# afanasyev-ilya/VectorGraphLibrary

Measured on AMD Instinct MI355X. Metric: TEPS (edges/s) BFS + SSSP on RMAT-24; value = direction-optimising BFS, sssp_value_teps = direction-optimising Bellman-Ford, higher is better.
Workload: dtype int32; 1 GPU; BFS direction-optimising on RMAT scale-24 (edge factor 32), 1xMI355X; vertices=16777216, edges=536870912, seed=1, parallelism=edge-cut x1, exchange_transport=none, vertex_numbering=degree-sorted (total)

## Files before the change

include/vgl_hip.h:

```cpp
#ifndef VGL_HIP_H
#define VGL_HIP_H
#include <stddef.h>
#include <stdint.h>
#ifdef __cplusplus
extern "C" {
#endif

#define VGL_HIP_ABI_VERSION 1

typedef struct vgl_hip_ctx vgl_hip_ctx;
typedef struct vgl_hip_graph vgl_hip_graph;
typedef struct vgl_hip_frontier vgl_hip_frontier;

int vgl_hip_abi_version(void);
const char *vgl_hip_last_error(void);
int vgl_hip_ctx_create(int device, void *stream, vgl_hip_ctx **out);
int vgl_hip_ctx_destroy(vgl_hip_ctx *ctx);
int vgl_hip_ctx_sync(vgl_hip_ctx *ctx);
int vgl_hip_ctx_trim(vgl_hip_ctx *ctx);
void *vgl_hip_ctx_stream(vgl_hip_ctx *ctx);

int vgl_hip_malloc(vgl_hip_ctx *ctx, size_t bytes, void **dptr);
int vgl_hip_free(vgl_hip_ctx *ctx, void *dptr);
int vgl_hip_memcpy_h2d(vgl_hip_ctx *ctx, void *dst, const void *src, size_t bytes);
// ... 267 lines not shown
    int64_t undirected_edges;
    int64_t components;
    int64_t bridges;
    int64_t articulation_points;
    int64_t biconnected_components;
    int64_t two_edge_components;
    int64_t largest_component_edges;
    int64_t algorithmic_bytes;
} vgl_hip_bicc_stats;
int vgl_hip_bicc_prepare(vgl_hip_ctx *ctx, vgl_hip_graph *g, int64_t *undirected_edges);
int vgl_hip_bicc_run(vgl_hip_ctx *ctx, vgl_hip_graph *g, int32_t *d_edge_u, int32_t *d_edge_v, uint8_t *d_bridge, int32_t *d_edge_component,
                     uint8_t *d_articulation, int32_t *d_two_edge_component, vgl_hip_bicc_stats *stats);

int vgl_hip_bfs_init(vgl_hip_ctx *ctx, int32_t V, int32_t source, int32_t *d_levels);
int vgl_hip_bfs_step_top_down(vgl_hip_ctx *ctx, vgl_hip_graph *g, int32_t *d_levels, int32_t level,
                              const uint64_t *d_visited_bits, int64_t *local_frontier, int64_t *local_edges);
int vgl_hip_bfs_step_top_down_bits(vgl_hip_ctx *ctx, vgl_hip_graph *graph, int32_t *d_levels, int32_t level,
                                   const uint64_t *d_visited_bits, const uint64_t *d_front_bits, uint64_t *d_next_bits,
                                   int64_t *local_frontier, int64_t *local_edges);
int vgl_hip_bitmap_or_parts(vgl_hip_ctx *ctx, int64_t words, int parts, const uint64_t *d_in, uint64_t *d_out);
int vgl_hip_bfs_step_bottom_up(vgl_hip_ctx *ctx, vgl_hip_graph *g, int32_t *d_levels, int32_t level,
                               const uint64_t *d_visited_bits, const uint64_t *d_front_bits, uint64_t *d_next_bits,
                               int64_t *found, int64_t *probed);
int vgl_hip_levels_to_bitmap(vgl_hip_ctx *ctx, int32_t V, const int32_t *d_levels, int32_t level, uint64_t *d_bits);
int vgl_hip_bfs_apply_bitmaps(vgl_hip_ctx *ctx, int32_t V, int parts, const uint64_t *d_bits_all, int32_t *d_levels, int32_t level,
                              uint64_t *d_visited_bits, uint64_t *d_front_bits, const int32_t *d_degrees, int64_t *newly,
                              int64_t *newly_degree);
int vgl_hip_bfs_apply_bitmaps_owned(vgl_hip_ctx *ctx, int32_t V, int parts, const uint64_t *d_bits_all, int32_t *d_levels, int32_t level,
                                    uint64_t *d_visited_bits, uint64_t *d_front_bits, const int32_t *d_degrees, int32_t own_begin,
                                    int32_t own_end, int64_t *newly_owned, int64_t *newly_owned_degree);
int vgl_hip_bitmap_to_ids(vgl_hip_ctx *ctx, int64_t words, const uint64_t *d_bits, int32_t cap, int32_t *d_out);
int vgl_hip_bfs_apply_ids(vgl_hip_ctx *ctx, int32_t V, int parts, int32_t cap, const int32_t *d_lists, int32_t *d_levels, int32_t level,
                          uint64_t *d_visited_bits, uint64_t *d_front_bits, const int32_t *d_degrees, int64_t *newly,
                          int64_t *newly_degree);
int vgl_hip_sssp_init(vgl_hip_ctx *ctx, int32_t V, int32_t source, float *d_dist);
int vgl_hip_sssp_relax_owned(vgl_hip_ctx *ctx, vgl_hip_graph *g, const float *d_weights, float *d_dist, int *changed);
int vgl_hip_cc_init(vgl_hip_ctx *ctx, int32_t V, int32_t *d_comp);
int vgl_hip_cc_hook_owned(vgl_hip_ctx *ctx, vgl_hip_graph *g, int32_t *d_comp, int *changed);
int vgl_hip_cc_jump(vgl_hip_ctx *ctx, int32_t V, int32_t *d_comp);
int vgl_hip_pr_setup(vgl_hip_ctx *ctx, int32_t V, const int32_t *d_indeg_noloops, float *d_ranks, float *d_rdeg);
int vgl_hip_sum_over_edges_f32(vgl_hip_ctx *ctx, vgl_hip_graph *g, const float *d_values, float sum_bound, float *d_sums);
int vgl_hip_pr_iteration_owned(vgl_hip_ctx *ctx, vgl_hip_graph *g, const int32_t *d_indeg_noloops, const float *d_rdeg,
                               float *d_ranks, float *d_contrib_scratch);
int vgl_hip_diff_to_pairs_u32(vgl_hip_ctx *ctx, int32_t n, const void *d_before, const void *d_after, int32_t cap, int32_t *d_out);
int vgl_hip_apply_pairs_u32(vgl_hip_ctx *ctx, int parts, int64_t stride, int skip_part, const int32_t *d_lists, int take_min, int32_t n,
                            void *d_values, int *changed);
// ... 55 lines not shown
```

vectorgraphlibrary_amd/api.py:

```python
import ctypes as C

import torch

from . import lib as _l

RMAT_ABCD = (57, 19, 19, 5)
BFS_TOP_DOWN, BFS_DIRECTION_OPT = 0, 1
SSSP_ALL_ACTIVE, SSSP_ACTIVE_TILES, SSSP_DELTA_STEPPING, SSSP_PULL, SSSP_DIRECTION_OPT = 0, 1, 2, 3, 4
DENSE, SPARSE, ALL_ACTIVE = 0, 1, 2
PR_EXACT_ORDER, PR_BLOCKED, PR_AUTO = 0, 1, 2
LP_ALL_ACTIVE, LP_FRONTIER, LP_AUTO = 0, 1, 2


def _ptr(t):
    return C.c_void_p(t.data_ptr()) if t is not None else None


class Context:

    def __init__(self, device=0):
        if not torch.cuda.is_available():
            raise _l.VglHipError("no HIP device visible: vectorgraphlibrary_amd has no CPU fallback")
        self.L = _l.load()
        self.device = torch.device("cuda", device)
# ... 4 lines not shown
        self.h = h

    def sync(self):
        _l.check(self.L.vgl_hip_ctx_sync(self.h))

    def close(self):
        if self.h:
            self.L.vgl_hip_ctx_destroy(self.h)
            self.h = None

    def empty(self, n, dtype):
        return torch.empty(int(n), dtype=dtype, device=self.device)

    def timing(self, enable=True, only=None, stride=1):
        _l.check(self.L.vgl_hip_timing_enable(self.h, int(enable)))
        _l.check(self.L.vgl_hip_timing_only(self.h, only.encode() if only else None))
        _l.check(self.L.vgl_hip_timing_stride(self.h, int(stride)))
        _l.check(self.L.vgl_hip_timing_reset(self.h))

    def timing_get(self, name):
        n, ms = C.c_int64(), C.c_double()
        _l.check(self.L.vgl_hip_timing_get(self.h, name.encode(), C.byref(n), C.byref(ms)))
        return n.value, ms.value

    def gen_rmat(self, scale, edge_factor, seed, relabel=True, first_edge=0, count=None):
        E = (1 << scale) * edge_factor if count is None else count
        src, dst = self.empty(E, torch.int32), self.empty(E, torch.int32)
        a, b, c, d = RMAT_ABCD
        _l.check(self.L.vgl_hip_gen_rmat(self.h, scale, first_edge, E, seed, a, b, c, d, int(relabel), _ptr(src), _ptr(dst)))
        return src, dst

    def gen_uniform(self, scale, edge_factor, seed, first_edge=0, count=None):
        E = (1 << scale) * edge_factor if count is None else count
        src, dst = self.empty(E, torch.int32), self.empty(E, torch.int32)
        _l.check(self.L.vgl_hip_gen_uniform(self.h, scale, first_edge, E, seed, _ptr(src), _ptr(dst)))
        return src, dst

    def gen_weights(self, E, seed, first_edge=0):
        w = self.empty(E, torch.float32)
        _l.check(self.L.vgl_hip_gen_weights(self.h, first_edge, E, seed, _ptr(w)))
        return w

    def coo_to_csr(self, V, src, dst, row_begin=0, row_end=None, want_perm=False):
        row_end = V if row_end is None else row_end
        E = src.numel()
        rowptr = self.empty(row_end - row_begin + 1, torch.int64)
# ... 627 lines not shown
```

vectorgraphlibrary_amd/csrc/bfs.hip:

```cpp
#include "vgl_hip_internal.h"
#include <chrono>
#include "vgl_gnf.h"
#include "vgl_blocked.h"

#ifndef VGL_BU_HEAVY_LANES
#define VGL_BU_HEAVY_LANES 16
#endif

__global__ __launch_bounds__(VGL_BLOCK) void vgl_k_bfs_init(int32_t V, int32_t source, int32_t *levels)
{
    for (int32_t v = blockIdx.x * VGL_BLOCK + threadIdx.x; v < V; v += gridDim.x * VGL_BLOCK)
        levels[v] = (v == source) ? 1 : -1;
}

__global__ __launch_bounds__(VGL_BLOCK) void vgl_k_bfs_init_all(int32_t V, int32_t source, int32_t *levels, int64_t words, uint64_t *visited,
                                                                uint64_t *front, uint64_t *next, uint32_t *tickets, unsigned long long *list_count)
{
    if (blockIdx.x == 0 && threadIdx.x == 0) *list_count = 0ULL;
    for (int32_t v = blockIdx.x * VGL_BLOCK + threadIdx.x; v < V; v += gridDim.x * VGL_BLOCK)
        levels[v] = (v == source) ? 1 : -1;
    for (int64_t w = (int64_t)blockIdx.x * VGL_BLOCK + threadIdx.x; w < words; w += (int64_t)gridDim.x * VGL_BLOCK) {
        const uint64_t bit = (w == (source >> 6)) ? (1ULL << (source & 63)) : 0ULL;
        visited[w] = bit; front[w] = bit; next[w] = 0;
    }
// ... 603 lines not shown
        host[C_NSLOTS] = seq;
        __threadfence_system();
    }
}

constexpr int VGL_BU_BLOCKS = 2048;

typedef int vgl_int4_u __attribute__((ext_vector_type(4), aligned(4)));

typedef unsigned vgl_uint3_u __attribute__((ext_vector_type(3), aligned(4)));
template <bool PACKED>
__device__ __forceinline__ void vgl_load_head(const int4 *in_head, int64_t rec, int32_t u[4])
{
    if constexpr (PACKED) {
        const vgl_uint3_u w = *reinterpret_cast<const vgl_uint3_u *>(reinterpret_cast<const uint32_t *>(in_head) + 3 * rec);
        const uint32_t f[4] = {w.x & 0xFFFFFFu, (w.x >> 24) | ((w.y & 0xFFFFu) << 8), (w.y >> 16) | ((w.z & 0xFFu) << 16), w.z >> 8};
#pragma unroll
        for (int q = 0; q < 4; q++) u[q] = f[q] == 0xFFFFFFu ? -1 : (int32_t)f[q];
    } else {
        const int4 h = in_head[rec];
        u[0] = h.x; u[1] = h.y; u[2] = h.z; u[3] = h.w;
    }
}
template <bool INLINE_HEAVY, bool PACKED>
__device__ __forceinline__ void vgl_bu_probe_body(int32_t nrows, int32_t row_base, int32_t chunk, const int64_t *in_rowptr,
                                                  const int32_t *in_adj, const uint64_t *visited, const uint64_t *in_nz,
                                                  const uint64_t *front, uint64_t *next, int32_t *levels, int32_t next_level,
                                                  int32_t *heavy, int64_t *partials, uint32_t *ticket, const int4 *in_head,
                                                  const uint64_t *in_long, const int32_t *nz_rank, int32_t nz_rows, int64_t *counters,
                                                  volatile int64_t *host, int64_t seq)
{
    static_assert(INLINE_HEAVY, "the deferred rows are scanned in the same launch");
    __shared__ int64_t s64[VGL_WAVES];
    __shared__ int s_nheavy;
    if (threadIdx.x == 0) s_nheavy = 0;
    __syncthreads();
    auto in_front = [&](int32_t u) -> uint32_t { return (uint32_t)((front[u >> 6] >> (u & 63)) & 1ULL); };
    int64_t found_cnt = 0, probes = 0;
    const int64_t groups = ((int64_t)nrows + 63) >> 6;
    const int64_t word0 = (int64_t)row_base >> 6;
    constexpr int64_t NW = (int64_t)VGL_BU_BLOCKS * VGL_WAVES;
    int32_t *my_heavy = heavy + (int64_t)blockIdx.x * chunk;
    const int lane = vgl_lane();
    for (int64_t g0 = (int64_t)blockIdx.x * VGL_WAVES + vgl_wave(); g0 < groups; g0 += NW * 64) {
        const int64_t mine = g0 + (int64_t)lane * NW;
        uint64_t cw = 0, nzw = 0;
        int32_t nzr = 0;
        if (mine < groups) {
            nzw = in_nz[word0 + mine];
            cw = ~visited[word0 + mine] & nzw;
            if (cw == 0ULL) next[word0 + mine] = 0ULL;
            else nzr = nz_rank[mine];
        }
        unsigned long long todo = __ballot(cw != 0ULL);
        while (todo) {
            const int j = __ffsll((long long)todo) - 1;
            todo &= todo - 1;
            const uint64_t cand_word = __shfl(cw, j);
            const int32_t rec = __shfl(nzr, j) + (int32_t)__popcll(__shfl(nzw, j) & ((1ULL << lane) - 1ULL));
            const int64_t grp = g0 + (int64_t)j * NW;
            const int32_t r = (int32_t)(grp << 6) + lane;
            const int32_t v = row_base + r;
            bool found = false, defer = false;
            if (r < nrows && ((cand_word >> lane) & 1ULL)) {
                int32_t u0[4];
                vgl_load_head<PACKED>(in_head, rec, u0);
                uint32_t hit = 0;
                int n = 0;
#pragma unroll
                for (int q = 0; q < 4; q++) if (u0[q] >= 0) n = q + 1;
                if (u0[0] >= 0) hit = in_front(u0[0]);
                if (hit == 0) {
#pragma unroll
                    for (int q = 1; q < 4; q++)
                        if (u0[q] >= 0) hit |= in_front(u0[q]) << q;
                }
                bool longer = false;
                if (hit == 0 && n == 4) {
                    int32_t u1[4];
                    vgl_load_head<PACKED>(in_head, (int64_t)nz_rows + rec, u1);
#pragma unroll
                    for (int q = 0; q < 4; q++)
                        if (u1[q] >= 0) { n = 5 + q; hit |= in_front(u1[q]) << (4 + q); }
                    longer = (in_long[v >> 6] >> (v & 63)) & 1ULL;
                }
                found = hit != 0;
                probes += found ? __ffs(hit) : n;
                defer = !found && longer;
                if (found) levels[v] = next_level;
            }
            const unsigned long long fm = __ballot(found);
            if (lane == 0) next[word0 + grp] = fm;
            found_cnt += found;
            const unsigned long long dm = __ballot(defer);
            if (dm) {
                int base = 0;
                if (lane == 0) base = atomicAdd(&s_nheavy, (int)__popcll(dm));
                base = __shfl(base, 0);
                if (defer) my_heavy[base + __popcll(dm & ((1ULL << lane) - 1ULL))] = r;
            }
        }
    }
    __syncthreads();
    const int nh = s_nheavy;
    constexpr int G = VGL_BU_HEAVY_LANES, NG = 64 / G;
    const int quarter = lane / G, ql = lane % G;
    for (int h0 = vgl_wave() * NG; h0 < nh; h0 += VGL_WAVES * NG) {
        const int h = h0 + quarter;
        bool done = h >= nh, hit_any = false;
        int32_t r = 0;
        int64_t p = 0, e = 0;
        if (!done) { r = my_heavy[h]; p = in_rowptr[r]; e = in_rowptr[r + 1]; }
        while (!__all(done)) {
            const int64_t q = p + ql;
            bool hit = false;
            if (!done && q < e) { const int32_t u = in_adj[q]; hit = (front[u >> 6] >> (u & 63)) & 1ULL; }
            const unsigned long long hm = __ballot(hit);
            const unsigned qm = (unsigned)(hm >> (quarter * G)) & (G >= 32 ? 0xFFFFFFFFu : ((1u << (G & 31)) - 1u));
            if (!done) {
                if (qm) { hit_any = true; done = true; if (ql == 0) probes += __ffs(qm); }
                else { if (ql == 0) probes += min((int64_t)G, e - p); p += G; if (p >= e) done = true; }
            }
        }
        if (hit_any && ql == 0) {
            const int32_t v = row_base + r;
            levels[v] = next_level;
            atomicOr((unsigned long long *)&next[v >> 6], 1ULL << (v & 63));
            found_cnt++;
        }
    }
    found_cnt = vgl_block_reduce_add(found_cnt, s64);
    probes = vgl_block_reduce_add(probes, s64);
    uint32_t dep = 0;
    if (threadIdx.x == 0) dep = vgl_put_agent(partials + blockIdx.x * 4 + 0, found_cnt) ^ vgl_put_agent(partials + blockIdx.x * 4 + 1, probes);
    if (!vgl_last_block(ticket, dep)) return;
    int64_t f = 0, pr = 0;
    for (int b = threadIdx.x; b < (int)gridDim.x; b += VGL_BLOCK) { f += vgl_load_agent(partials + b * 4 + 0); pr += vgl_load_agent(partials + b * 4 + 1); }
    f = vgl_block_reduce_add(f, s64);
    pr = vgl_block_reduce_add(pr, s64);
    if (threadIdx.x == 0) {
        if (host) vgl_publish2(counters, host, seq, C_BU_FOUND, f, C_BU_EDGES, pr);
        else { counters[C_BU_FOUND] = f; counters[C_BU_EDGES] = pr; }
    }
}
#define VGL_BU_PROBE_PARAMS                                                                                                                             \
    int32_t nrows, int32_t row_base, int32_t chunk, const int64_t *in_rowptr, const int32_t *in_adj, const uint64_t *visited, const uint64_t *in_nz,  \
        const uint64_t *front, uint64_t *next, int32_t *levels, int32_t next_level, int32_t *heavy, int64_t *partials, uint32_t *ticket,               \
        const int4 *in_head, const uint64_t *in_long, const int32_t *nz_rank, int32_t nz_rows, int64_t *counters, volatile int64_t *host, int64_t seq
#define VGL_BU_PROBE_ARGS                                                                                                                               \
    nrows, row_base, chunk, in_rowptr, in_adj, visited, in_nz, front, next, levels, next_level, heavy, partials, ticket, in_head, in_long, nz_rank,    \
        nz_rows, counters, host, seq
template <bool INLINE_HEAVY>
__global__ __launch_bounds__(VGL_BLOCK) __attribute__((amdgpu_num_sgpr(80))) void vgl_k_bu_probe(VGL_BU_PROBE_PARAMS)
{
    vgl_bu_probe_body<INLINE_HEAVY, true>(VGL_BU_PROBE_ARGS);
}
template <bool INLINE_HEAVY>
__global__ __launch_bounds__(VGL_BLOCK) void vgl_k_bu_probe_wide(VGL_BU_PROBE_PARAMS)
{
    vgl_bu_probe_body<INLINE_HEAVY, false>(VGL_BU_PROBE_ARGS);
}

__global__ __launch_bounds__(VGL_BLOCK) void vgl_k_bm_advance(int64_t words, uint64_t *visited, uint64_t *front, uint64_t *next)
{
    for (int64_t w = (int64_t)blockIdx.x * VGL_BLOCK + threadIdx.x; w < words; w += (int64_t)gridDim.x * VGL_BLOCK) {
        const uint64_t n = next[w];
        if (n) { visited[w] |= n; next[w] = 0; }
        front[w] = n;
    }
}

constexpr int VGL_B2I_BLOCKS = 2048;
__global__ __launch_bounds__(VGL_BLOCK) void vgl_k_bitmap_to_ids(int64_t words, const uint64_t *bits, int64_t word_base, int32_t cap, int32_t *out)
{
    __shared__ int s32[VGL_WAVES];
    __shared__ int s_base;
    const int64_t per = (((words + gridDim.x - 1) / gridDim.x + VGL_BLOCK - 1) / VGL_BLOCK) * VGL_BLOCK;
    const int64_t lo = (int64_t)blockIdx.x * per, hi = min(words, lo + per);
    int n = 0;
    for (int64_t wi = lo + threadIdx.x; wi < hi; wi += VGL_BLOCK) n += (int)__popcll(bits[wi]);
    int total = 0;
    vgl_block_excl_add(n, s32, &total);
    if (total == 0) return;
    if (threadIdx.x == 0) s_base = atomicAdd(out, total);
// ... 156 lines not shown
            if (advance)
                hipLaunchKernelGGL(vgl_k_bm_gnf_count<true>, dim3(nb), dim3(VGL_BLOCK), 0, c->stream, nwords, word0, g->row_begin, g->bm_front,
                                   g->out.rowptr, g->vt_cnt, g->vt_deg, g->vt_cnt_off, g->vt_deg_off, g->offs, c->d_counters,
                                   g->tickets + 0 * VGL_TICKET_WORDS, (volatile int64_t *)c->h_counters, seq, g->bm_visited, g->bm_next,
                                   hint ? 1 : 0, hint ? *hint : no_hint);
            else
                hipLaunchKernelGGL(vgl_k_bm_gnf_count<false>, dim3(nb), dim3(VGL_BLOCK), 0, c->stream, nwords, word0, g->row_begin,
                                   const_cast<uint64_t *>(front), g->out.rowptr, g->vt_cnt, g->vt_deg, g->vt_cnt_off, g->vt_deg_off, g->offs, c->d_counters,
                                   g->tickets + 0 * VGL_TICKET_WORDS, (volatile int64_t *)c->h_counters, seq, (uint64_t *)nullptr, (uint64_t *)nullptr,
                                   0, no_hint);
        }
        VGL_HIP_TRY(hipGetLastError());
        VGL_TRY(vgl_wait_counters(c, seq));
    }
    if (write) {
        vgl_timed_launch tl(c, "gnf");
        hipLaunchKernelGGL(vgl_k_bm_gnf_write, dim3(nb), dim3(VGL_BLOCK), 0, c->stream, nwords, word0, g->row_begin, front,
                           g->out.rowptr, g->vt_cnt_off, g->vt_deg_off, g->ids, g->offs, g->tile_first, M_known >= 0 ? M_known : c->h_counters[C_NEIGH]);
        VGL_HIP_TRY(hipGetLastError());
    }
    return 0;
}

static int vgl_bfs_bu_launch(vgl_hip_ctx *c, vgl_hip_graph *g, int32_t *levels, int32_t next_level, const uint64_t *visited,
                             const uint64_t *front, uint64_t *next, int64_t *seq_out)
{
    const int32_t chunk = (int32_t)(vgl_ceil_div(vgl_ceil_div(g->nrows, VGL_BU_BLOCKS), VGL_BLOCK) * VGL_BLOCK);
    const int64_t seq = vgl_next_seq(c);
    {
        vgl_timed_launch tl(c, "bfs_bottom_up");
        auto *kernel = g->in_head_packed ? vgl_k_bu_probe<true> : vgl_k_bu_probe_wide<true>;
        hipLaunchKernelGGL(kernel, dim3(VGL_BU_BLOCKS), dim3(VGL_BLOCK), 0, c->stream, g->nrows, g->row_begin, chunk,
                           g->in.rowptr, g->in.adj, visited, g->bm_in_nz, front, next, levels, next_level, g->heavy, g->bu_partials,
                           g->tickets + 1 * VGL_TICKET_WORDS, reinterpret_cast<const int4 *>(g->in_head.p), g->bm_in_long,
                           (const int32_t *)g->in_nz_rank, g->in_nz_rows, c->d_counters, (volatile int64_t *)c->h_counters, seq);
    }
    VGL_HIP_TRY(hipGetLastError());
    if (seq_out) *seq_out = seq;
    return 0;
}

static int vgl_bfs_blocked_level(vgl_hip_ctx *c, vgl_hip_graph *g, int32_t *levels, int32_t next_level)
{
    for (const vgl_blocked_piece &p : g->blk_bfs->pieces) {
        if (p.n_g_units > 0) {
            vgl_timed_launch tl(c, "bfs_blk_gather");
            hipLaunchKernelGGL(vgl_k_bfs_blk_gather, dim3((unsigned)p.n_g_units), dim3(VGL_BTHREADS), 0, c->stream, (const vgl_blk_unit *)p.g_units,
                               (const uint16_t *)p.g_lo, (const uint32_t *)p.mid_to_a, reinterpret_cast<uint64_t *>(p.vals.p), p.g_count,
                               (const uint64_t *)g->bm_front, (int64_t)g->row_begin >> 6);
        }
        if (p.n_a_units > 0) {
            vgl_timed_launch tl(c, "bfs_blk_accumulate");
// ... 19 lines not shown
}

int vgl_bitmap_to_ids(vgl_hip_ctx *c, int64_t words, const uint64_t *d_bits, int64_t word_base, int32_t cap, int32_t *d_out)
{
    VGL_HIP_TRY(hipMemsetAsync(d_out, 0, sizeof(int32_t), c->stream));
    if (words > 0) {
        vgl_timed_launch tl(c, "bfs_shard_resolve");
        hipLaunchKernelGGL(vgl_k_bitmap_to_ids, dim3((unsigned)std::min<int64_t>(VGL_B2I_BLOCKS, vgl_ceil_div(words, VGL_BLOCK))), dim3(VGL_BLOCK), 0, c->stream,
                           words, d_bits, word_base, cap, d_out);
    }
    VGL_HIP_TRY(hipGetLastError());
    return 0;
}

static int64_t vgl_bfs_td_emit_edges(int64_t V) { return std::max<int64_t>(65536, V / 256); }

struct vgl_bfs_params {
    int64_t td_emit_edges;
    double td_filter_share;
    double td_late_share;
    double blocked_share;
    int64_t small_m;
    int64_t bm_expand_f;
    bool use_hints, scan_bound, trace;
};
static vgl_bfs_params vgl_bfs_params_of(const vgl_bfs_tunables &tn, int64_t V, int mode)
{
    const bool do_mode = mode == VGL_HIP_BFS_DIRECTION_OPT;
    vgl_bfs_params p;
    p.td_emit_edges = tn.td_emit_edges >= 0 ? tn.td_emit_edges : vgl_bfs_td_emit_edges(V);
    p.td_filter_share = tn.td_filter_share >= 0.0 ? tn.td_filter_share : 0.125;
    p.td_late_share = tn.td_late_share >= 0.0 ? tn.td_late_share : 1.0 / 64;
    p.blocked_share = tn.blocked_share >= 0.0 ? tn.blocked_share : 0.1;
    p.small_m = tn.small_m >= 0 ? std::min<int64_t>(tn.small_m, 1 << 20) : 8192;
    if (do_mode) p.small_m = std::min<int64_t>(p.small_m, vgl_do_bottom_up_edges(V, V, 1) - 1);
    if (p.small_m < 64) p.small_m = 0;
    p.bm_expand_f = tn.bm_expand >= 0 ? tn.bm_expand : 262144;
    if (vgl_ceil_div(vgl_ceil_div(V, 64), VGL_BLOCK) > 8192) p.bm_expand_f = 0;
    p.use_hints = do_mode && !tn.no_hint;
    p.scan_bound = do_mode && !tn.no_scan_bound;
    p.trace = tn.trace;
    return p;
}

enum class vgl_bfs_front {
    levels,
    pending,
    bitmap,
    counted_bitmap,
    counted_scan,
    ids,
};

struct vgl_bfs_traversal {
    vgl_hip_ctx *c;
    vgl_hip_graph *g;
    int mode;
    int32_t *levels;
    vgl_bfs_params p;
    int32_t V;
    int64_t E, words, factor;
// ... 157 lines not shown
            VGL_TRY(small_levels((int32_t)F, -1, false));
            trace("list kernel done");
            book_small(F);
            return 0;
        }
        const bool is_late = late();
        const bool emit = M <= p.td_emit_edges || is_late;
        const bool td_counts = emit && p.use_hints && vgl_ceil_div(M, VGL_TILE) <= VGL_TD_COUNT_TILES;
        const bool filter = is_late || (double)visited_total >= p.td_filter_share * (double)V;
        trace(emit ? "counted + ids -> top-down (emitting)" : "counted + ids -> top-down (levels only)");
        VGL_TRY(vgl_bfs_td_launch(c, g, (int32_t)F, M, levels, cur + 1, emit, have_tile_first, td_counts, filter));
        trace("top-down done");
        hint_ready = td_counts && F > 0 && M > 0;
        front = emit ? vgl_bfs_front::pending : vgl_bfs_front::levels;
        book_top_down(F, M);
        cur++;
        return 0;
    }
    int bottom_up_level()
    {
        if (front == vgl_bfs_front::levels || front == vgl_bfs_front::pending) VGL_FAIL("bfs_run: internal error (bitmaps missing)");
        int64_t seq = 0;
        trace("-> bottom-up");
        VGL_TRY(vgl_bfs_bu_launch(c, g, levels, cur + 1, g->bm_visited, g->bm_front, g->bm_next, &seq));
        hipLaunchKernelGGL(vgl_k_bm_advance, dim3(vgl_grid(words, VGL_BLOCK, 8192)), dim3(VGL_BLOCK), 0, c->stream, words, g->bm_visited, g->bm_front, g->bm_next);
        VGL_HIP_TRY(hipGetLastError());
        VGL_TRY(vgl_wait_counters(c, seq));
        st.bu_steps++; st.edges_examined += c->h_counters[C_BU_EDGES];
        st.bu_edges += c->h_counters[C_BU_EDGES]; st.bu_found += c->h_counters[C_BU_FOUND];
        F = c->h_counters[C_BU_FOUND]; M = 0;
        front = vgl_bfs_front::bitmap;
        cur++;
        return 0;
    }

    int run(int32_t source)
    {
        hipLaunchKernelGGL(vgl_k_bfs_init_all, dim3(vgl_grid(V, VGL_BLOCK, 8192)), dim3(VGL_BLOCK), 0, c->stream, V, source, levels, words, g->bm_visited, g->bm_front,
                           g->bm_next, g->tickets, list_count);
        t0 = std::chrono::steady_clock::now();
        if (p.small_m > 0) {
            VGL_TRY(small_levels(1, source, false));
            if (c->h_counters[C_TMP0] > 0) {
                begin_level(1);
                prevF = 1;
                book_small(1);
            }
// ... 121 lines not shown
        vgl_timed_launch tl(c, "gnf");
        hipLaunchKernelGGL(vgl_k_levels_to_bitmap<false>, dim3(vgl_grid(g->V, VGL_BLOCK, 8192)), dim3(VGL_BLOCK), 0, c->stream, g->V, (const int32_t *)d_levels, level + 1, d_next_bits);
    }
    VGL_HIP_TRY(hipGetLastError());
    return 0;
}

int vgl_hip_bfs_step_bottom_up(vgl_hip_ctx *c, vgl_hip_graph *g, int32_t *d_levels, int32_t level, const uint64_t *d_visited_bits,
                               const uint64_t *d_front_bits, uint64_t *d_next_bits, int64_t *found, int64_t *probed)
{
    if (!c || !g || !d_levels || !d_visited_bits || !d_front_bits || !d_next_bits) VGL_FAIL("bfs_step_bottom_up: null argument");
    if (!g->in.rowptr) VGL_FAIL("bfs_step_bottom_up: the incoming CSR of the owned rows is required");
    VGL_TRY(vgl_zero_words(c, d_next_bits, vgl_ceil_div(g->V, 64)));
    int64_t seq = 0;
    VGL_TRY(vgl_bfs_bu_launch(c, g, d_levels, level + 1, d_visited_bits, d_front_bits, d_next_bits, &seq));
    if (found || probed) {
        VGL_TRY(vgl_wait_counters(c, seq));
        if (found) *found = c->h_counters[C_BU_FOUND];
        if (probed) *probed = c->h_counters[C_BU_EDGES];
    }
    return 0;
}

int vgl_hip_bitmap_or_parts(vgl_hip_ctx *c, int64_t words, int parts, const uint64_t *d_in, uint64_t *d_out)
{
    if (!c || !d_in || !d_out) VGL_FAIL("bitmap_or_parts: null argument");
    if (words < 0 || parts < 1) VGL_FAIL("bitmap_or_parts: bad size");
    if (words > 0) hipLaunchKernelGGL(vgl_k_bitmap_or_parts, dim3(vgl_grid(words, VGL_BLOCK, 8192)), dim3(VGL_BLOCK), 0, c->stream, words, parts, d_in, d_out);
    VGL_HIP_TRY(hipGetLastError());
    return 0;
}

int vgl_hip_levels_to_bitmap(vgl_hip_ctx *c, int32_t V, const int32_t *d_levels, int32_t level, uint64_t *d_bits)
{
    if (!c || !d_levels || !d_bits) VGL_FAIL("levels_to_bitmap: null argument");
    hipLaunchKernelGGL(vgl_k_levels_to_bitmap<false>, dim3(vgl_grid(V, VGL_BLOCK, 8192)), dim3(VGL_BLOCK), 0, c->stream, V, d_levels, level, d_bits);
    VGL_HIP_TRY(hipGetLastError());
    return 0;
}

int vgl_hip_bitmap_to_ids(vgl_hip_ctx *c, int64_t words, const uint64_t *d_bits, int32_t cap, int32_t *d_out)
{
    if (!c || !d_bits || !d_out) VGL_FAIL("bitmap_to_ids: null argument");
    if (words < 0 || cap < 1) VGL_FAIL("bitmap_to_ids: bad size");
    return vgl_bitmap_to_ids(c, words, d_bits, 0, cap, d_out);
}
// ... 63 lines not shown
```

vectorgraphlibrary_amd/csrc/context.hip:

```cpp
#include "vgl_hip_internal.h"
#include <unordered_set>
#include <cstdio>
#include <cstring>
#include <mutex>
#include <algorithm>

static thread_local std::string g_last_error;

int vgl_set_error(const char *file, int line, const char *msg)
{
    char buf[512];
    const char *base = strrchr(file, '/');
    snprintf(buf, sizeof(buf), "vgl_hip: %s (%s:%d)", msg, base ? base + 1 : file, line);
    g_last_error = buf;
    return 1;
}

static hipMemPool_t g_lib_pool[64];
static bool g_lib_pool_tried[64];
static std::mutex g_lib_pool_mutex;
hipMemPool_t vgl_lib_pool(int device)
{
    if (device < 0 || device >= 64) return nullptr;
    std::lock_guard<std::mutex> lock(g_lib_pool_mutex);
// ... 29 lines not shown
extern char **environ;
static uint64_t vgl_env_signature()
{
    uint64_t h = 1469598103934665603ull ^ (uint64_t)(uintptr_t)environ;
    if (environ) for (char **e = environ; *e; e++) h = (h ^ (uint64_t)(uintptr_t)*e) * 1099511628211ull;
    return h ? h : 1;
}
void vgl_ctx_refresh_env(vgl_hip_ctx *c)
{
    const uint64_t sig = vgl_env_signature();
    if (sig == c->env_signature) return;
    c->env_signature = sig;
    c->env.clear();
    if (environ)
        for (char **e = environ; *e; e++)
            if (strncmp(*e, "VGL_", 4) == 0)
                if (const char *eq = strchr(*e, '=')) c->env[std::string(*e, (size_t)(eq - *e))] = std::string(eq + 1);
    vgl_bfs_tunables t;
    auto str = [&](const char *n) -> const char * { auto it = c->env.find(n); return it == c->env.end() ? nullptr : it->second.c_str(); };
    auto on = [&](const char *n) { const char *v = str(n); return v && v[0] == '1'; };
    if (const char *v = str("VGL_TD_EMIT_EDGES")) t.td_emit_edges = atoll(v);
    if (const char *v = str("VGL_BFS_SMALL_M")) t.small_m = atoll(v);
    if (const char *v = str("VGL_BFS_BM_EXPAND")) t.bm_expand = atoll(v);
    if (const char *v = str("VGL_SHARD_TD_EMIT_EDGES")) t.shard_td_emit_edges = atoll(v);
    if (const char *v = str("VGL_TD_FILTER_SHARE")) t.td_filter_share = atof(v);
    if (const char *v = str("VGL_TD_LATE_SHARE")) t.td_late_share = atof(v);
    if (const char *v = str("VGL_BFS_BLOCKED_SHARE")) t.blocked_share = atof(v);
    if (const char *v = str("VGL_SHARD_SPARSE_CAP")) t.shard_sparse_cap = std::max(0, atoi(v));
    t.no_hint = on("VGL_BFS_NO_HINT"); t.no_scan_bound = on("VGL_BFS_NO_SCAN_BOUND"); t.trace = on("VGL_BFS_TRACE");
    c->bfs = t;
}
const char *vgl_env(vgl_hip_ctx *c, const char *name)
{
    vgl_ctx_refresh_env(c);
    auto it = c->env.find(name);
    return it == c->env.end() ? nullptr : it->second.c_str();
}
int64_t vgl_env_int(vgl_hip_ctx *c, const char *name, int64_t dflt, int64_t lo, int64_t hi)
{
    const char *s = vgl_env(c, name);
    const int64_t v = (s && *s) ? strtoll(s, nullptr, 10) : dflt;
    return std::min(hi, std::max(lo, v));
}

extern "C" {

// ... 241 lines not shown
```

vectorgraphlibrary_amd/csrc/graph_frontier.hip:

```cpp
#include "vgl_hip_internal.h"
#include <atomic>
#include "vgl_gnf.h"
#include "vgl_blocked.h"

__global__ __launch_bounds__(VGL_BLOCK) void vgl_k_tile_rows(int32_t nrows, const int64_t *rowptr, int32_t *tile_row, int64_t ntiles)
{
    for (int32_t r = blockIdx.x * VGL_BLOCK + threadIdx.x; r < nrows; r += gridDim.x * VGL_BLOCK) {
        const int64_t t0 = (rowptr[r] + VGL_TILE - 1) / VGL_TILE;
        const int64_t t1 = (rowptr[r + 1] + VGL_TILE - 1) / VGL_TILE;
        for (int64_t t = t0; t < t1; t++) tile_row[t] = r;
        if (rowptr[r] < rowptr[r + 1] && rowptr[r + 1] == rowptr[nrows]) tile_row[ntiles] = r;
    }
}

__global__ __launch_bounds__(VGL_BLOCK) void vgl_k_nonempty_rows(int32_t nrows, int32_t row_base, const int64_t *rowptr, uint64_t *bits)
{
    const int32_t nround = (nrows + 63) & ~63;
    for (int32_t r = blockIdx.x * VGL_BLOCK + threadIdx.x; r < nround; r += gridDim.x * VGL_BLOCK) {
        const bool on = r < nrows && rowptr[r + 1] > rowptr[r];
        const unsigned long long m = __ballot(on);
        if ((threadIdx.x & 63) == 0) bits[(row_base + r) >> 6] = m;
    }
}

// ... 259 lines not shown
                         const int64_t *d_in_rowptr, const int32_t *d_in_adj, int64_t in_edges, vgl_hip_graph **out)
{
    if (!c || !out) VGL_FAIL("graph_create: null argument");
    if (V <= 0) VGL_FAIL("graph_create: vertices_count must be positive");
    if (row_begin < 0 || row_end > V || row_begin >= row_end) VGL_FAIL("graph_create: bad owned row range");
    if (row_begin % 64 != 0) VGL_FAIL("graph_create: row_begin must be a multiple of 64 (use vgl_hip_partition_rows)");
    if (!d_out_rowptr || (!d_out_adj && out_edges > 0)) VGL_FAIL("graph_create: outgoing CSR is required");
    if (out_edges < 0 || in_edges < 0) VGL_FAIL("graph_create: negative edge count");
    VGL_HIP_TRY(hipSetDevice(c->device));
    vgl_building<vgl_hip_graph> g(new vgl_hip_graph(), {c});
    static std::atomic<uint64_t> next_uid{1};
    g->uid = next_uid.fetch_add(1);
    g->V = V; g->row_begin = row_begin; g->row_end = row_end; g->nrows = row_end - row_begin;
    g->out.rowptr = d_out_rowptr; g->out.adj = d_out_adj; g->out.edges = out_edges;
    VGL_TRY(vgl_build_tile_rows(c, g->out, g->nrows));
    if (d_in_rowptr) {
        g->in.rowptr = d_in_rowptr; g->in.adj = d_in_adj; g->in.edges = in_edges;
        VGL_TRY(vgl_build_tile_rows(c, g->in, g->nrows));
    }
    const size_t words = (size_t)vgl_ceil_div(V, 64) + 1;
    VGL_TRY(g->bm_visited.alloc(words));
    VGL_TRY(g->bm_front.alloc(words));
    VGL_TRY(g->bm_next.alloc(words));
    VGL_TRY(g->bm_in_nz.alloc(words));
    VGL_TRY(g->ids.alloc((size_t)g->nrows));
    VGL_TRY(g->offs.alloc((size_t)g->nrows + 1));
    g->nvtiles = vgl_ceil_div(g->nrows, VGL_TILE);
    VGL_TRY(g->vt_cnt.alloc((size_t)g->nvtiles));
    VGL_TRY(g->vt_cnt_off.alloc((size_t)g->nvtiles));
    VGL_TRY(g->vt_deg.alloc((size_t)g->nvtiles));
    VGL_TRY(g->vt_deg_off.alloc((size_t)g->nvtiles));
    VGL_TRY(g->vt_min_deg.alloc((size_t)g->nvtiles));
    hipLaunchKernelGGL(vgl_k_tile_min_degree, dim3((unsigned)g->nvtiles), dim3(VGL_BLOCK), 0, c->stream, g->nrows, g->out.rowptr, g->vt_min_deg);
    VGL_TRY(g->tile_first.alloc((size_t)g->out.ntiles + 2));
    VGL_TRY(g->heavy.alloc((size_t)g->nrows + 4096 * VGL_BLOCK));
    VGL_TRY(g->bu_partials.alloc((size_t)4096 * 4));
    VGL_TRY(g->tickets.alloc((size_t)4 * VGL_TICKET_WORDS));
    VGL_HIP_TRY(hipMemsetAsync(g->tickets, 0, 4 * VGL_TICKET_WORDS * sizeof(uint32_t), c->stream));
    VGL_TRY(g->epoch.alloc((size_t)V));
    VGL_TRY(g->fscratch.alloc((size_t)V));
    VGL_TRY(g->fscratch2.alloc((size_t)V));
    VGL_TRY(g->fscratch3.alloc((size_t)V));
    VGL_TRY(g->iscratch.alloc((size_t)V));
    VGL_HIP_TRY(hipMemsetAsync(g->bm_visited, 0, words * 8, c->stream));
    VGL_HIP_TRY(hipMemsetAsync(g->bm_front, 0, words * 8, c->stream));
    VGL_HIP_TRY(hipMemsetAsync(g->bm_next, 0, words * 8, c->stream));
// ... 351 lines not shown
```

vectorgraphlibrary_amd/csrc/vgl_hip_internal.h:

```cpp
#pragma once
#include <hip/hip_runtime.h>
#include <stdint.h>
#include <string>
#include <map>
#include <memory>
#include <vector>
#include "../../include/vgl_hip.h"

constexpr int VGL_BLOCK = 256;
constexpr int VGL_EPT = 8;
constexpr int VGL_TILE = VGL_BLOCK * VGL_EPT;
constexpr int VGL_WAVES = VGL_BLOCK / 64;

int vgl_set_error(const char *file, int line, const char *msg);
#define VGL_FAIL(msg) return vgl_set_error(__FILE__, __LINE__, (msg))
#define VGL_HIP_TRY(expr)                                                          \
    do {                                                                           \
        hipError_t _e = (expr);                                                    \
        if (_e != hipSuccess) return vgl_set_error(__FILE__, __LINE__, hipGetErrorString(_e)); \
    } while (0)
#define VGL_TRY(expr)            \
    do {                         \
        int _s = (expr);         \
        if (_s != 0) return _s;  \
    } while (0)

enum {
    C_FRONT = 0, C_NEIGH = 1, C_BU_FOUND = 2, C_BU_EDGES = 3, C_HEAVY = 4, C_CHANGED = 5,
    C_EDGES = 6, C_TMP0 = 7, C_TMP1 = 8, C_JUMP = 9,
    C_NEXT_F = 10, C_NEXT_M = 11,
    C_SKIPPED = 12, C_HINT = 13,
    C_NSLOTS = 32
};
constexpr int VGL_NSHARD = 1024;

struct vgl_timing_slot {
    int64_t launches = 0;
    std::vector<std::pair<hipEvent_t, hipEvent_t>> pending;
    double total_ms = 0.0;
};

struct vgl_bfs_tunables {
    int64_t td_emit_edges = -1, small_m = -1, bm_expand = -1, shard_td_emit_edges = -1;
    double td_filter_share = -1.0, td_late_share = -1.0, blocked_share = -1.0;
    int shard_sparse_cap = -1;
    bool no_hint = false, no_scan_bound = false, trace = false;
};

struct vgl_hip_ctx {
    std::map<std::string, std::string> env;
    uint64_t env_signature = 0;
    vgl_bfs_tunables bfs;
    int device = 0;
    hipStream_t stream = nullptr;
    bool own_stream = false;
    int64_t *d_counters = nullptr;
    int64_t *d_shards = nullptr;
    int64_t *h_counters = nullptr;
    int64_t publish_seq = 0;
    double *d_partials = nullptr;
    size_t partials_cap = 0;
    bool timing = false;
    std::string timing_only;
    int timing_stride = 1;
    int64_t timing_seen = 0;
    std::map<std::string, vgl_timing_slot> slots;
// ... 75 lines not shown
    vgl_dev<int32_t> tile_row;
    int64_t ntiles = 0;
    vgl_dev<int32_t> hub_rows;
    int32_t nhubs = 0;
    int hub_blocks = 0;
    vgl_dev<int32_t> giant_rows;
    int ngiants = 0, giant_blocks = 0;
    vgl_dev<int32_t> hub_chunks;
    int n_hub_chunks = 0, n_hub_list = 0;
    vgl_dev<double> hub_chunk_sums;
    vgl_dev<int32_t> pull_blk_row;
    int pull_nblk = 0;
    int64_t max_row = -1;
};

template <class T> void vgl_cache_free(T *p);
template <class T> struct vgl_cache_delete { void operator()(T *p) const { vgl_cache_free(p); } };
template <class T> using vgl_cache = std::unique_ptr<T, vgl_cache_delete<T>>;
struct vgl_hip_graph {
    uint64_t uid = 0;
    int32_t V = 0, row_begin = 0, row_end = 0, nrows = 0;
    vgl_dir_csr out, in;
    vgl_dev<uint64_t> bm_visited, bm_front, bm_next;
    vgl_dev<uint64_t> bm_in_nz;
    vgl_dev<int32_t> in_head;
    bool in_head_packed = false;
    vgl_dev<int32_t> in_nz_rank;
    int32_t in_nz_rows = 0;
    vgl_dev<int32_t> pr_indeg;
    bool pr_indeg_ready = false;
    vgl_dev<uint64_t> bm_in_long;
    vgl_dev<int32_t> ids;
    vgl_dev<int64_t> offs;
    vgl_dev<int32_t> vt_cnt, vt_cnt_off;
    vgl_dev<int64_t> vt_deg, vt_deg_off;
    int64_t nvtiles = 0;
    vgl_dev<int32_t> vt_min_deg;
    vgl_dev<uint8_t> gnf_bits;
    vgl_dev<int32_t> tile_first;
    vgl_dev<int32_t> heavy;
    vgl_dev<int64_t> bu_partials;
    vgl_dev<uint32_t> tickets;
    vgl_dev<int32_t> epoch;
    vgl_dev<float> fscratch;
    vgl_dev<float> fscratch2;
    vgl_dev<float> fscratch3;
// ... 259 lines not shown
```

vectorgraphlibrary_amd/lib.py:

```python
import ctypes as C
import os

_HERE = os.path.dirname(os.path.abspath(__file__))
LIB_PATH = os.path.join(_HERE, "libvgl_hip.so")


class VglHipError(RuntimeError):
    pass


class BfsStats(C.Structure):
    _fields_ = [("levels", C.c_int32), ("td_steps", C.c_int32), ("bu_steps", C.c_int32),
                ("edges_examined", C.c_int64), ("frontier_total", C.c_int64), ("discovered", C.c_int64),
                ("algorithmic_bytes", C.c_int64), ("td_edges", C.c_int64), ("td_frontier", C.c_int64),
                ("bu_edges", C.c_int64), ("bu_found", C.c_int64)]


class SsspStats(C.Structure):
    _fields_ = [("iterations", C.c_int32), ("edges_relaxed", C.c_int64), ("algorithmic_bytes", C.c_int64),
                ("push_steps", C.c_int32), ("pull_steps", C.c_int32)]


class PrStats(C.Structure):
    _fields_ = [("iterations", C.c_int32), ("ranks_sum", C.c_double), ("algorithmic_bytes", C.c_int64)]
# ... 129 lines not shown
    "vgl_hip_cc_run": [_p, _p, _p, C.POINTER(CcStats)],
    "vgl_hip_cc_run_symmetric": [_p, _p, _p, C.POINTER(CcStats)],
    "vgl_hip_lp_prepare": [_p, _p, _int],
    "vgl_hip_lp_run": [_p, _p, _int, _int, _int, _int, _p, _p, C.POINTER(_i64), C.POINTER(LpStats)],
    "vgl_hip_tri_prepare": [_p, _p],
    "vgl_hip_tri_run": [_p, _p, C.POINTER(_i64), _p, _p, C.POINTER(TriStats)],
    "vgl_hip_bc_prepare": [_p, _p, _int],
    "vgl_hip_bc_run": [_p, _p, C.POINTER(_i32), _i32, _int, _int, _p, _p, _p, _p, C.POINTER(BcStats)],
    "vgl_hip_msbfs_prepare": [_p, _p, _int, _int],
    "vgl_hip_msbfs_run": [_p, _p, C.POINTER(_i32), _i32, _int, _int, _p, _p, _p, _p, _p, C.POINTER(MsbfsStats)],
    "vgl_hip_kcore_prepare": [_p, _p],
    "vgl_hip_kcore_run": [_p, _p, _i32, _p, _p, C.POINTER(KcoreStats)],
    "vgl_hip_ktruss_prepare": [_p, _p, C.POINTER(_i64)],
    "vgl_hip_ktruss_run": [_p, _p, _i32, _p, _p, _p, _p, C.POINTER(KtrussStats)],
    "vgl_hip_msf_prepare": [_p, _p, C.POINTER(_i64)],
    "vgl_hip_msf_run": [_p, _p, _p, _p, _p, _p, _p, _p, C.POINTER(MsfStats)],
    "vgl_hip_bicc_prepare": [_p, _p, C.POINTER(_i64)],
    "vgl_hip_bicc_run": [_p, _p, _p, _p, _p, _p, _p, _p, C.POINTER(BiccStats)],
    "vgl_hip_bfs_init": [_p, _i32, _i32, _p],
    "vgl_hip_bfs_step_top_down": [_p, _p, _p, _i32, _p, C.POINTER(_i64), C.POINTER(_i64)],
    "vgl_hip_bfs_step_top_down_bits": [_p, _p, _p, _i32, _p, _p, _p, C.POINTER(_i64), C.POINTER(_i64)],
    "vgl_hip_bitmap_or_parts": [_p, _i64, _int, _p, _p],
    "vgl_hip_bfs_step_bottom_up": [_p, _p, _p, _i32, _p, _p, _p, C.POINTER(_i64), C.POINTER(_i64)],
    "vgl_hip_levels_to_bitmap": [_p, _i32, _p, _i32, _p],
    "vgl_hip_bfs_apply_bitmaps": [_p, _i32, _int, _p, _p, _i32, _p, _p, _p, C.POINTER(_i64), C.POINTER(_i64)],
    "vgl_hip_bfs_apply_bitmaps_owned": [_p, _i32, _int, _p, _p, _i32, _p, _p, _p, _i32, _i32, C.POINTER(_i64), C.POINTER(_i64)],
    "vgl_hip_bitmap_to_ids": [_p, _i64, _p, _i32, _p],
    "vgl_hip_bfs_apply_ids": [_p, _i32, _int, _i32, _p, _p, _i32, _p, _p, _p, C.POINTER(_i64), C.POINTER(_i64)],
    "vgl_hip_sssp_init": [_p, _i32, _i32, _p],
    "vgl_hip_sssp_relax_owned": [_p, _p, _p, _p, C.POINTER(_int)],
    "vgl_hip_sswp_init": [_p, _i32, _i32, _p],
    "vgl_hip_sswp_relax_owned": [_p, _p, _p, _p, C.POINTER(_int)],
    "vgl_hip_cc_init": [_p, _i32, _p],
    "vgl_hip_cc_hook_owned": [_p, _p, _p, C.POINTER(_int)],
    "vgl_hip_cc_jump": [_p, _i32, _p],
    "vgl_hip_pr_setup": [_p, _i32, _p, _p, _p],
    "vgl_hip_sum_over_edges_f32": [_p, _p, _p, C.c_float, _p],
    "vgl_hip_sssp_prepare": [_p, _p],
    "vgl_hip_comm_set_timeout_ms": [_p, C.c_double],
    "vgl_hip_pr_iteration_owned": [_p, _p, _p, _p, _p, _p],
    "vgl_hip_indegree_noloops_add": [_p, _p, _p],
    "vgl_hip_diff_to_pairs_u32": [_p, _i32, _p, _p, _i32, _p],
    "vgl_hip_apply_pairs_u32": [_p, _int, _i64, _int, _p, _int, _i32, _p, C.POINTER(_int)],
    "vgl_hip_comm_unique_id": [_p],
    "vgl_hip_comm_create": [_p, _int, _int, _p, _pp],
    "vgl_hip_comm_create_hosted": [_p, _int, _int, C.c_char_p, C.c_size_t, _pp],
# ... 64 lines not shown
```

Before: 1809 billion edges/s.

## Filter bottom-up frontier probes through a folded shared-memory frontier summary

When the frontier is small (F at or below a threshold, default 65536), a new kernel ORs the frontier bitmap into a 2048-word fold. The bottom-up probe kernels load this fold into LDS and only read the global frontier word when the folded bit is set, which is meant to cut random global loads on sparse frontiers. The cost is an extra kernel launch, an LDS preload per block, and extra branching in the probe path. False positives from hash collisions still fall through to the real frontier check, so results stay exact.

```diff
diff --git a/include/vgl_hip.h b/include/vgl_hip.h
--- a/include/vgl_hip.h
+++ b/include/vgl_hip.h
@@ -313,6 +313,7 @@
 int vgl_hip_bfs_step_bottom_up(vgl_hip_ctx *ctx, vgl_hip_graph *g, int32_t *d_levels, int32_t level,
                                const uint64_t *d_visited_bits, const uint64_t *d_front_bits, uint64_t *d_next_bits,
                                int64_t *found, int64_t *probed);
+int vgl_hip_bfs_front_fold(vgl_hip_ctx *ctx, int64_t words, const uint64_t *d_front, uint64_t *d_fold);
 int vgl_hip_levels_to_bitmap(vgl_hip_ctx *ctx, int32_t V, const int32_t *d_levels, int32_t level, uint64_t *d_bits);
 int vgl_hip_bfs_apply_bitmaps(vgl_hip_ctx *ctx, int32_t V, int parts, const uint64_t *d_bits_all, int32_t *d_levels, int32_t level,
                               uint64_t *d_visited_bits, uint64_t *d_front_bits, const int32_t *d_degrees, int64_t *newly,
diff --git a/vectorgraphlibrary_amd/api.py b/vectorgraphlibrary_amd/api.py
--- a/vectorgraphlibrary_amd/api.py
+++ b/vectorgraphlibrary_amd/api.py
@@ -50,6 +50,12 @@
         n, ms = C.c_int64(), C.c_double()
         _l.check(self.L.vgl_hip_timing_get(self.h, name.encode(), C.byref(n), C.byref(ms)))
         return n.value, ms.value
+
+    def bfs_front_fold(self, front, words=None):
+        words = front.numel() if words is None else int(words)
+        fold = self.empty(2048, torch.int64)
+        _l.check(self.L.vgl_hip_bfs_front_fold(self.h, words, _ptr(front), _ptr(fold)))
+        return fold
 
     def gen_rmat(self, scale, edge_factor, seed, relabel=True, first_edge=0, count=None):
         E = (1 << scale) * edge_factor if count is None else count
diff --git a/vectorgraphlibrary_amd/csrc/bfs.hip b/vectorgraphlibrary_amd/csrc/bfs.hip
--- a/vectorgraphlibrary_amd/csrc/bfs.hip
+++ b/vectorgraphlibrary_amd/csrc/bfs.hip
@@ -649,20 +649,41 @@
         u[0] = h.x; u[1] = h.y; u[2] = h.z; u[3] = h.w;
     }
 }
-template <bool INLINE_HEAVY, bool PACKED>
+template <bool INLINE_HEAVY, bool PACKED, bool FILTER = false>
 __device__ __forceinline__ void vgl_bu_probe_body(int32_t nrows, int32_t row_base, int32_t chunk, const int64_t *in_rowptr,
                                                   const int32_t *in_adj, const uint64_t *visited, const uint64_t *in_nz,
                                                   const uint64_t *front, uint64_t *next, int32_t *levels, int32_t next_level,
                                                   int32_t *heavy, int64_t *partials, uint32_t *ticket, const int4 *in_head,
                                                   const uint64_t *in_long, const int32_t *nz_rank, int32_t nz_rows, int64_t *counters,
-                                                  volatile int64_t *host, int64_t seq)
+                                                  volatile int64_t *host, int64_t seq, const uint64_t *fold = nullptr)
 {
     static_assert(INLINE_HEAVY, "the deferred rows are scanned in the same launch");
     __shared__ int64_t s64[VGL_WAVES];
     __shared__ int s_nheavy;
+    __shared__ uint64_t s_fold[FILTER ? VGL_FOLD_WORDS : 1];
     if (threadIdx.x == 0) s_nheavy = 0;
+    if constexpr (FILTER) {
+#pragma unroll
+        for (int i = 0; i < VGL_FOLD_WORDS / VGL_BLOCK; i++) s_fold[i * VGL_BLOCK + threadIdx.x] = fold[i * VGL_BLOCK + threadIdx.x];
+    }
     __syncthreads();
-    auto in_front = [&](int32_t u) -> uint32_t { return (uint32_t)((front[u >> 6] >> (u & 63)) & 1ULL); };
+    [[maybe_unused]] auto folded = [&](int32_t u) -> bool { return (s_fold[(u >> 6) & (VGL_FOLD_WORDS - 1)] >> (u & 63)) & 1ULL; };
+    auto in_front = [&](int32_t u) -> uint32_t {
+        if constexpr (FILTER) {
+            if (!folded(u)) return 0u;
+        }
+        return (uint32_t)((front[u >> 6] >> (u & 63)) & 1ULL);
+    };
+    [[maybe_unused]] auto in_front4 = [&](const int32_t u[4], int q0) -> uint32_t {
+        uint64_t w[4] = {0ULL, 0ULL, 0ULL, 0ULL};
+#pragma unroll
+        for (int q = 0; q < 4; q++)
+            if (q >= q0 && u[q] >= 0 && folded(u[q])) w[q] = front[u[q] >> 6];
+        uint32_t hit = 0;
+#pragma unroll
+        for (int q = 0; q < 4; q++) hit |= (uint32_t)((w[q] >> (u[q] & 63)) & 1ULL) << q;
+        return hit;
+    };
     int64_t found_cnt = 0, probes = 0;
     const int64_t groups = ((int64_t)nrows + 63) >> 6;
     const int64_t word0 = (int64_t)row_base >> 6;
@@ -698,17 +719,26 @@
                 for (int q = 0; q < 4; q++) if (u0[q] >= 0) n = q + 1;
                 if (u0[0] >= 0) hit = in_front(u0[0]);
                 if (hit == 0) {
-#pragma unroll
-                    for (int q = 1; q < 4; q++)
-                        if (u0[q] >= 0) hit |= in_front(u0[q]) << q;
+                    if constexpr (FILTER) hit = in_front4(u0, 1);
+                    else {
+#pragma unroll
+                        for (int q = 1; q < 4; q++)
+                            if (u0[q] >= 0) hit |= in_front(u0[q]) << q;
+                    }
                 }
                 bool longer = false;
                 if (hit == 0 && n == 4) {
                     int32_t u1[4];
                     vgl_load_head<PACKED>(in_head, (int64_t)nz_rows + rec, u1);
-#pragma unroll
-                    for (int q = 0; q < 4; q++)
-                        if (u1[q] >= 0) { n = 5 + q; hit |= in_front(u1[q]) << (4 + q); }
+                    if constexpr (FILTER) {
+#pragma unroll
+                        for (int q = 0; q < 4; q++) if (u1[q] >= 0) n = 5 + q;
+                        hit = in_front4(u1, 0) << 4;
+                    } else {
+#pragma unroll
+                        for (int q = 0; q < 4; q++)
+                            if (u1[q] >= 0) { n = 5 + q; hit |= in_front(u1[q]) << (4 + q); }
+                    }
                     longer = (in_long[v >> 6] >> (v & 63)) & 1ULL;
                 }
                 found = hit != 0;
@@ -741,7 +771,7 @@
         while (!__all(done)) {
             const int64_t q = p + ql;
             bool hit = false;
-            if (!done && q < e) { const int32_t u = in_adj[q]; hit = (front[u >> 6] >> (u & 63)) & 1ULL; }
+            if (!done && q < e) hit = in_front(in_adj[q]) != 0;
             const unsigned long long hm = __ballot(hit);
             const unsigned qm = (unsigned)(hm >> (quarter * G)) & (G >= 32 ? 0xFFFFFFFFu : ((1u << (G & 31)) - 1u));
             if (!done) {
@@ -787,6 +817,37 @@
 {
     vgl_bu_probe_body<INLINE_HEAVY, false>(VGL_BU_PROBE_ARGS);
 }
+template <bool INLINE_HEAVY>
+__global__ __launch_bounds__(VGL_BLOCK) __attribute__((amdgpu_num_sgpr(80))) void vgl_k_bu_probe_filtered(VGL_BU_PROBE_PARAMS, const uint64_t *fold)
+{
+    vgl_bu_probe_body<INLINE_HEAVY, true, true>(VGL_BU_PROBE_ARGS, fold);
+}
+template <bool INLINE_HEAVY>
+__global__ __launch_bounds__(VGL_BLOCK) void vgl_k_bu_probe_wide_filtered(VGL_BU_PROBE_PARAMS, const uint64_t *fold)
+{
+    vgl_bu_probe_body<INLINE_HEAVY, false, true>(VGL_BU_PROBE_ARGS, fold);
+}
+
+constexpr int VGL_FOLD_COLS = 16, VGL_FOLD_SLICES = VGL_BLOCK / VGL_FOLD_COLS;
+__global__ __launch_bounds__(VGL_BLOCK) void vgl_k_front_fold(int64_t words, const uint64_t *front, uint64_t *fold)
+{
+    __shared__ uint64_t s_part[VGL_WAVES][VGL_FOLD_COLS];
+    const int col = threadIdx.x % VGL_FOLD_COLS, slice = threadIdx.x / VGL_FOLD_COLS;
+    const int64_t j = (int64_t)blockIdx.x * VGL_FOLD_COLS + col;
+    uint64_t acc = 0;
+    for (int64_t w = j + (int64_t)slice * VGL_FOLD_WORDS; w < words; w += (int64_t)VGL_FOLD_SLICES * VGL_FOLD_WORDS) acc |= front[w];
+    acc |= __shfl_xor(acc, 16);
+    acc |= __shfl_xor(acc, 32);
+    if (vgl_lane() < VGL_FOLD_COLS) s_part[vgl_wave()][col] = acc;
+    __syncthreads();
+    if (threadIdx.x < VGL_FOLD_COLS) {
+        uint64_t r = 0;
+#pragma unroll
+        for (int w = 0; w < VGL_WAVES; w++) r |= s_part[w][threadIdx.x];
+        fold[j] = r;
+    }
+}
+static_assert(VGL_FOLD_WORDS % VGL_FOLD_COLS == 0 && VGL_FOLD_COLS == 16 && VGL_BLOCK == 256, "vgl_k_front_fold: 16 columns, 4 slices per wavefront");
 
 __global__ __launch_bounds__(VGL_BLOCK) void vgl_k_bm_advance(int64_t words, uint64_t *visited, uint64_t *front, uint64_t *next)
 {
@@ -989,12 +1050,27 @@
     return 0;
 }
 
+static int vgl_front_fold_launch(vgl_hip_ctx *c, int64_t words, const uint64_t *front, uint64_t *fold)
+{
+    vgl_timed_launch tl(c, "bfs_front_fold");
+    hipLaunchKernelGGL(vgl_k_front_fold, dim3(VGL_FOLD_WORDS / VGL_FOLD_COLS), dim3(VGL_BLOCK), 0, c->stream, words, front, fold);
+    return 0;
+}
 static int vgl_bfs_bu_launch(vgl_hip_ctx *c, vgl_hip_graph *g, int32_t *levels, int32_t next_level, const uint64_t *visited,
-                             const uint64_t *front, uint64_t *next, int64_t *seq_out)
+                             const uint64_t *front, uint64_t *next, int64_t *seq_out, bool filtered = false)
 {
     const int32_t chunk = (int32_t)(vgl_ceil_div(vgl_ceil_div(g->nrows, VGL_BU_BLOCKS), VGL_BLOCK) * VGL_BLOCK);
     const int64_t seq = vgl_next_seq(c);
-    {
+    if (filtered) {
+        VGL_TRY(vgl_front_fold_launch(c, vgl_ceil_div(g->V, 64), front, g->bm_fold));
+        vgl_timed_launch tl(c, "bfs_bottom_up");
+        auto *kernel = g->in_head_packed ? vgl_k_bu_probe_filtered<true> : vgl_k_bu_probe_wide_filtered<true>;
+        hipLaunchKernelGGL(kernel, dim3(VGL_BU_BLOCKS), dim3(VGL_BLOCK), 0, c->stream, g->nrows, g->row_begin, chunk,
+                           g->in.rowptr, g->in.adj, visited, g->bm_in_nz, front, next, levels, next_level, g->heavy, g->bu_partials,
+                           g->tickets + 1 * VGL_TICKET_WORDS, reinterpret_cast<const int4 *>(g->in_head.p), g->bm_in_long,
+                           (const int32_t *)g->in_nz_rank, g->in_nz_rows, c->d_counters, (volatile int64_t *)c->h_counters, seq,
+                           (const uint64_t *)g->bm_fold);
+    } else {
         vgl_timed_launch tl(c, "bfs_bottom_up");
         auto *kernel = g->in_head_packed ? vgl_k_bu_probe<true> : vgl_k_bu_probe_wide<true>;
         hipLaunchKernelGGL(kernel, dim3(VGL_BU_BLOCKS), dim3(VGL_BLOCK), 0, c->stream, g->nrows, g->row_begin, chunk,
@@ -1060,6 +1136,7 @@
     double blocked_share;
     int64_t small_m;
     int64_t bm_expand_f;
+    int64_t filter_f;
     bool use_hints, scan_bound, trace;
 };
 static vgl_bfs_params vgl_bfs_params_of(const vgl_bfs_tunables &tn, int64_t V, int mode)
@@ -1075,6 +1152,7 @@
     if (p.small_m < 64) p.small_m = 0;
     p.bm_expand_f = tn.bm_expand >= 0 ? tn.bm_expand : 262144;
     if (vgl_ceil_div(vgl_ceil_div(V, 64), VGL_BLOCK) > 8192) p.bm_expand_f = 0;
+    p.filter_f = tn.filter_f >= 0 ? tn.filter_f : 65536;
     p.use_hints = do_mode && !tn.no_hint;
     p.scan_bound = do_mode && !tn.no_scan_bound;
     p.trace = tn.trace;
@@ -1278,7 +1356,9 @@
         if (front == vgl_bfs_front::levels || front == vgl_bfs_front::pending) VGL_FAIL("bfs_run: internal error (bitmaps missing)");
         int64_t seq = 0;
         trace("-> bottom-up");
-        VGL_TRY(vgl_bfs_bu_launch(c, g, levels, cur + 1, g->bm_visited, g->bm_front, g->bm_next, &seq));
+        const bool filtered = F <= p.filter_f;
+        if (filtered) trace("bottom-up through the folded frontier");
+        VGL_TRY(vgl_bfs_bu_launch(c, g, levels, cur + 1, g->bm_visited, g->bm_front, g->bm_next, &seq, filtered));
         hipLaunchKernelGGL(vgl_k_bm_advance, dim3(vgl_grid(words, VGL_BLOCK, 8192)), dim3(VGL_BLOCK), 0, c->stream, words, g->bm_visited, g->bm_front, g->bm_next);
         VGL_HIP_TRY(hipGetLastError());
         VGL_TRY(vgl_wait_counters(c, seq));
@@ -1446,6 +1526,15 @@
     return 0;
 }
 
+int vgl_hip_bfs_front_fold(vgl_hip_ctx *c, int64_t words, const uint64_t *d_front, uint64_t *d_fold)
+{
+    if (!c || !d_fold || (!d_front && words > 0)) VGL_FAIL("bfs_front_fold: null argument");
+    if (words < 0) VGL_FAIL("bfs_front_fold: bad size");
+    VGL_TRY(vgl_front_fold_launch(c, words, d_front, d_fold));
+    VGL_HIP_TRY(hipGetLastError());
+    return 0;
+}
+
 int vgl_hip_bitmap_or_parts(vgl_hip_ctx *c, int64_t words, int parts, const uint64_t *d_in, uint64_t *d_out)
 {
     if (!c || !d_in || !d_out) VGL_FAIL("bitmap_or_parts: null argument");
diff --git a/vectorgraphlibrary_amd/csrc/context.hip b/vectorgraphlibrary_amd/csrc/context.hip
--- a/vectorgraphlibrary_amd/csrc/context.hip
+++ b/vectorgraphlibrary_amd/csrc/context.hip
@@ -75,6 +75,7 @@
     if (const char *v = str("VGL_TD_EMIT_EDGES")) t.td_emit_edges = atoll(v);
     if (const char *v = str("VGL_BFS_SMALL_M")) t.small_m = atoll(v);
     if (const char *v = str("VGL_BFS_BM_EXPAND")) t.bm_expand = atoll(v);
+    if (const char *v = str("VGL_BFS_FILTER_F")) t.filter_f = atoll(v);
     if (const char *v = str("VGL_SHARD_TD_EMIT_EDGES")) t.shard_td_emit_edges = atoll(v);
     if (const char *v = str("VGL_TD_FILTER_SHARE")) t.td_filter_share = atof(v);
     if (const char *v = str("VGL_TD_LATE_SHARE")) t.td_late_share = atof(v);
diff --git a/vectorgraphlibrary_amd/csrc/graph_frontier.hip b/vectorgraphlibrary_amd/csrc/graph_frontier.hip
--- a/vectorgraphlibrary_amd/csrc/graph_frontier.hip
+++ b/vectorgraphlibrary_amd/csrc/graph_frontier.hip
@@ -305,6 +305,7 @@
     VGL_TRY(g->bm_visited.alloc(words));
     VGL_TRY(g->bm_front.alloc(words));
     VGL_TRY(g->bm_next.alloc(words));
+    VGL_TRY(g->bm_fold.alloc((size_t)VGL_FOLD_WORDS));
     VGL_TRY(g->bm_in_nz.alloc(words));
     VGL_TRY(g->ids.alloc((size_t)g->nrows));
     VGL_TRY(g->offs.alloc((size_t)g->nrows + 1));
diff --git a/vectorgraphlibrary_amd/csrc/vgl_hip_internal.h b/vectorgraphlibrary_amd/csrc/vgl_hip_internal.h
--- a/vectorgraphlibrary_amd/csrc/vgl_hip_internal.h
+++ b/vectorgraphlibrary_amd/csrc/vgl_hip_internal.h
@@ -11,6 +11,7 @@
 constexpr int VGL_EPT = 8;
 constexpr int VGL_TILE = VGL_BLOCK * VGL_EPT;
 constexpr int VGL_WAVES = VGL_BLOCK / 64;
+constexpr int VGL_FOLD_WORDS = 2048;
 
 int vgl_set_error(const char *file, int line, const char *msg);
 #define VGL_FAIL(msg) return vgl_set_error(__FILE__, __LINE__, (msg))
@@ -41,7 +42,7 @@
 };
 
 struct vgl_bfs_tunables {
-    int64_t td_emit_edges = -1, small_m = -1, bm_expand = -1, shard_td_emit_edges = -1;
+    int64_t td_emit_edges = -1, small_m = -1, bm_expand = -1, shard_td_emit_edges = -1, filter_f = -1;
     double td_filter_share = -1.0, td_late_share = -1.0, blocked_share = -1.0;
     int shard_sparse_cap = -1;
     bool no_hint = false, no_scan_bound = false, trace = false;
@@ -163,6 +164,7 @@
     int32_t V = 0, row_begin = 0, row_end = 0, nrows = 0;
     vgl_dir_csr out, in;
     vgl_dev<uint64_t> bm_visited, bm_front, bm_next;
+    vgl_dev<uint64_t> bm_fold;
     vgl_dev<uint64_t> bm_in_nz;
     vgl_dev<int32_t> in_head;
     bool in_head_packed = false;
diff --git a/vectorgraphlibrary_amd/lib.py b/vectorgraphlibrary_amd/lib.py
--- a/vectorgraphlibrary_amd/lib.py
+++ b/vectorgraphlibrary_amd/lib.py
@@ -175,6 +175,7 @@
     "vgl_hip_bfs_step_top_down_bits": [_p, _p, _p, _i32, _p, _p, _p, C.POINTER(_i64), C.POINTER(_i64)],
     "vgl_hip_bitmap_or_parts": [_p, _i64, _int, _p, _p],
     "vgl_hip_bfs_step_bottom_up": [_p, _p, _p, _i32, _p, _p, _p, C.POINTER(_i64), C.POINTER(_i64)],
+    "vgl_hip_bfs_front_fold": [_p, _i64, _p, _p],
     "vgl_hip_levels_to_bitmap": [_p, _i32, _p, _i32, _p],
     "vgl_hip_bfs_apply_bitmaps": [_p, _i32, _int, _p, _p, _i32, _p, _p, _p, C.POINTER(_i64), C.POINTER(_i64)],
     "vgl_hip_bfs_apply_bitmaps_owned": [_p, _i32, _int, _p, _p, _i32, _p, _p, _p, _i32, _i32, C.POINTER(_i64), C.POINTER(_i64)],
```

Result: faster. 1865 billion edges/s (median of 6 runs) (+3.1%).
